# aproposorg/sydr

Hardware: AMD Instinct MI355X
Metric: IQ Msamples/s through 32-ch E/P/L correlators @25 MHz fs (higher is better)
Workload: dtype f64

## Files before the change

### sydr_amd/csrc/engine.hip

```cpp
#include "engine_internal.h"
#include <sched.h>
#include <cstdint>
#include <cerrno>
#include <cctype>
#include "build_id.h"

#include <cstring>

static thread_local std::string g_last_error = "";

void sdr_set_error(const char* fmt, ...) {
    char buf[1024];
    va_list ap;
    va_start(ap, fmt);
    vsnprintf(buf, sizeof(buf), fmt, ap);
    va_end(ap);
    g_last_error = buf;
}

int sdr_fail(int status, const char* fmt, ...) {
    char buf[1024];
    va_list ap;
    va_start(ap, fmt);
    vsnprintf(buf, sizeof(buf), fmt, ap);
    va_end(ap);
    g_last_error = buf;
    return status;
}

int sdr_set_device_keep(sdr_engine* e) {
    if (!e) return sdr_fail(SDR_ERR_INVALID, "engine is NULL");
    SDR_HIP(hipSetDevice(e->device));
    return SDR_OK;
}

int sdr_set_device(sdr_engine* e) {
    if (int rc = sdr_set_device_keep(e)) return rc;
    e->srv_steady_ticks = 0;
    if (e->srv_running)
        if (int rc = sdr_tick_server_stop(e)) return rc;
    e->last_tick_took_slab = false;
    if (e->srv_slab_pending)
        if (int rc = sdr_iq_flush_server_slab(e)) return rc;
    return SDR_OK;
}

int sdr_devbuf_reserve(sdr_engine* e, DevBuf* b, size_t bytes) { return sdr_devbuf_reserve_on(e, e->stream, b, bytes); }

int sdr_pinned_reserve(sdr_engine* e, StreamCtx* ctx, size_t bytes) {
    if (bytes <= ctx->pinned_bytes && ctx->pinned) return SDR_OK;
    if (ctx->pinned) {
        SDR_HIP(hipStreamSynchronize(ctx->stream));
        SDR_HIP(hipHostFree(ctx->pinned));
        ctx->pinned = nullptr;
        ctx->pinned_bytes = 0;
    }
    const size_t want = bytes < 65536 ? 65536 : bytes * 2;
    hipError_t err = hipHostMalloc(&ctx->pinned, want, hipHostMallocDefault);
    if (err != hipSuccess) {
        ctx->pinned = nullptr;
        return sdr_fail(SDR_ERR_NOMEM, "hipHostMalloc(%zu) failed: %s", want, hipGetErrorString(err));
    }
    ctx->pinned_bytes = want;
    (void)e;
    return SDR_OK;
}

StreamCtx* sdr_stream_ctx(sdr_engine* e, int stream_id) {
    if (stream_id == 0) return &e->ctx0;
    if (stream_id < 0 || stream_id > (int)e->streams.size()) return nullptr;
    return e->streams[(size_t)stream_id - 1];
}

int sdr_devbuf_reserve_on(sdr_engine* e, hipStream_t stream, DevBuf* b, size_t bytes) {
    (void)e;
    if (bytes <= b->bytes && b->ptr) return SDR_OK;
    if (b->ptr) {
        SDR_HIP(hipStreamSynchronize(stream));
        SDR_HIP(hipFree(b->ptr));
        b->ptr = nullptr;
        b->bytes = 0;
    }
    size_t want = bytes < 256 ? 256 : bytes;
    hipError_t err = hipMalloc(&b->ptr, want);
    if (err != hipSuccess) {
        b->ptr = nullptr;
        return sdr_fail(SDR_ERR_NOMEM, "hipMalloc(%zu) failed: %s", want, hipGetErrorString(err));
    }
    b->bytes = want;
    return SDR_OK;
}

ProfScope::ProfScope(sdr_engine* eng, const char* name, hipStream_t on)
    : e(eng), active(eng->prof), stream(on ? on : eng->stream) {
    rec.name = name;
    rec.start = rec.stop = nullptr;
    if (active && e->prof_calls_only != (strncmp(name, "call_", 5) == 0)) active = false;
    if (!active) return;
    for (int i = 0; i < 2; ++i) {
        hipEvent_t ev = nullptr;
        if (!e->prof_pool.empty()) {
            ev = e->prof_pool.back();
            e->prof_pool.pop_back();
        } else if (hipEventCreate(&ev) != hipSuccess) {
            active = false;
            return;
        }
        (i == 0 ? rec.start : rec.stop) = ev;
    }
    (void)hipEventRecord(rec.start, stream);
}

ProfScope::~ProfScope() {
    if (!active) return;
    (void)hipEventRecord(rec.stop, stream);
    e->prof_records.push_back(rec);
}

__global__ __launch_bounds__(256) void hbm_copy_kernel(const uint4* __restrict__ src, uint4* __restrict__ dst, size_t n16) {
    const size_t stride = (size_t)gridDim.x * blockDim.x;
    size_t i = (size_t)blockIdx.x * blockDim.x + threadIdx.x;
    for (; i + 3 * stride < n16; i += 4 * stride) {
        const uint4 a = src[i], b = src[i + stride], c = src[i + 2 * stride], d = src[i + 3 * stride];
        dst[i] = a;
        dst[i + stride] = b;
// ... 76 lines not shown
    if (have_saved) now = saved;
    int n = 0;
    for (char* p = list; got && *p && *p != '\n';) {
        char* end = nullptr;
        const long a = strtol(p, &end, 10);
        if (end == p) break;
        long b = a;
        p = end;
        if (*p == '-') {
            b = strtol(p + 1, &end, 10);
            p = end;
        }
        for (long c = a; c <= b && c < CPU_SETSIZE; ++c)
            if (c >= 0 && CPU_ISSET((int)c, &now)) CPU_SET((int)c, &want), ++n;
        if (*p == ',') ++p;
    }
    if (!n) return sdr_fail(SDR_ERR_UNSUPPORTED, "%s names no CPU this thread may run on ('%s')", path, list);
    if (!have_saved) saved = now, have_saved = true;
    if (sched_setaffinity(0, sizeof(want), &want) != 0) return sdr_fail(SDR_ERR_UNSUPPORTED, "sched_setaffinity: %s", strerror(errno));
    return SDR_OK;
}

extern "C" {

int sdr_set_option(sdr_engine* e, const char* name, int value) {
    if (!e || !name) return sdr_fail(SDR_ERR_INVALID, "NULL engine or option name");
    if (!strcmp(name, "pcps_materialise_map")) e->pcps_force_map = value != 0;
    else if (!strcmp(name, "pcps_general_kernels")) e->pcps_no_fast = value != 0;
    else if (!strcmp(name, "pcps_one_stream")) e->pcps_no_overlap = value != 0;
    else if (!strcmp(name, "pcps_fused")) e->pcps_fused = value != 0;
    else if (!strcmp(name, "pcps_no_spectra_cache")) e->pcps_no_spec_cache = value != 0;
    else if (!strcmp(name, "ingest_by_copy_command")) e->ingest_by_copy = value != 0;
    else if (!strcmp(name, "track_one_launch_tick")) e->track_one_launch_tick = value != 0;
    else if (!strcmp(name, "track_two_launch_tick")) e->track_two_launch_tick = value != 0;
    else if (!strcmp(name, "ingest_with_tick")) e->ingest_with_tick = value != 0;
    else if (!strcmp(name, "pcps_no_shared_spectra")) e->pcps_no_shared_spectra = value != 0;
    else if (!strcmp(name, "tick_server")) {
        if (int rc = sdr_set_device_keep(e)) return rc;
        if (e->srv_running) (void)sdr_tick_server_stop(e);
        e->tick_server_opt = value != 0;
    }
    else if (!strcmp(name, "bind_thread_to_device")) return bind_thread_to_device(e, value);
    else if (!strcmp(name, "pcps_prn_chunk")) e->pcps_prn_chunk = value;
    else if (!strcmp(name, "coherent_scratch_kb")) {
        if (value < 0) return sdr_fail(SDR_ERR_RANGE, "coherent_scratch_kb %d is negative", value);
        e->coh_scratch_kb = value;
    }
    else if (!strcmp(name, "epl_no_chip_variant")) e->epl_no_chip = value != 0;
    else if (!strcmp(name, "epl_no_split_variant")) e->epl_no_split = value != 0;
    else if (!strcmp(name, "epl_xcd_run")) {
        if (value < -1 || value > kEplXcdRunMax) return sdr_fail(SDR_ERR_RANGE, "epl_xcd_run %d outside -1..%d", value, kEplXcdRunMax);
        e->epl_xcd_run = value < 0 ? kEplXcdRunDefault : value;
    }
    else if (!strcmp(name, "epl_no_half_chip_view")) e->epl_no_double = value != 0;
    else if (!strcmp(name, "epl_no_two_chip_variant")) e->epl_no_chip2 = value != 0;
    else if (!strcmp(name, "corr_profile_per_sample")) e->corr_per_sample = value != 0;
    else if (!strcmp(name, "ddm_per_sample")) e->ddm_per_sample = value != 0;
    else return sdr_fail(SDR_ERR_INVALID, "unknown option '%s'", name);
    return SDR_OK;
}

int sdr_hbm_copy_rate(sdr_engine* e, int64_t n_bytes, int reps, double* gbps) {
    if (int rc = sdr_set_device(e)) return rc;
    if (!gbps || n_bytes < (1 << 20) || reps < 1) return sdr_fail(SDR_ERR_INVALID, "bad copy-rate request");
    const size_t n16 = (size_t)n_bytes / 16;
    void *a = nullptr, *b = nullptr;
    hipError_t err = hipMalloc(&a, n16 * 16);
    if (err == hipSuccess) err = hipMalloc(&b, n16 * 16);
    if (err != hipSuccess) {
        if (a) (void)hipFree(a);
        return sdr_fail(SDR_ERR_NOMEM, "hipMalloc for the copy test failed: %s", hipGetErrorString(err));
    }
    hipEvent_t t0, t1;
    SDR_HIP(hipEventCreate(&t0));
    SDR_HIP(hipEventCreate(&t1));
    SDR_HIP(hipMemsetAsync(a, 1, n16 * 16, e->stream));
    const int blocks = e->n_cus * 8;
    hipLaunchKernelGGL(hbm_copy_kernel, dim3(blocks), dim3(256), 0, e->stream, (const uint4*)a, (uint4*)b, n16);
    SDR_HIP(hipEventRecord(t0, e->stream));
    for (int r = 0; r < reps; ++r)
        hipLaunchKernelGGL(hbm_copy_kernel, dim3(blocks), dim3(256), 0, e->stream, (const uint4*)a, (uint4*)b, n16);
    SDR_HIP(hipEventRecord(t1, e->stream));
    SDR_HIP(hipStreamSynchronize(e->stream));
    float ms = 0.f;
    SDR_HIP(hipEventElapsedTime(&ms, t0, t1));
    (void)hipEventDestroy(t0);
    (void)hipEventDestroy(t1);
    (void)hipFree(a);
    (void)hipFree(b);
    *gbps = 2.0 * (double)(n16 * 16) * reps / (ms * 1e-3) / 1e9;
    return SDR_OK;
}

const char* sdr_last_error(void) { return g_last_error.c_str(); }

int sdr_abi_version(void) { return SDR_ABI_VERSION; }
const char* sdr_build_id(void) { return SDR_BUILD_ID; }

int sdr_device_count(int* n) {
    if (!n) return sdr_fail(SDR_ERR_INVALID, "n is NULL");
    int c = 0;
    hipError_t err = hipGetDeviceCount(&c);
    if (err != hipSuccess) {
        (void)hipGetLastError();
        c = 0;
    }
// ... 22 lines not shown
    sdr_engine* e = new (std::nothrow) sdr_engine();
    if (!e) return sdr_fail(SDR_ERR_NOMEM, "host allocation failed");
    e->device = device_id;
    e->n_cus = prop.multiProcessorCount;
    err = hipStreamCreateWithFlags(&e->stream, hipStreamNonBlocking);
    if (err != hipSuccess) {
        delete e;
        return sdr_fail(SDR_ERR_HIP, "hipStreamCreate failed: %s", hipGetErrorString(err));
    }
    e->ctx0.stream = e->stream;
    *out = e;
    return SDR_OK;
}

static void free_ctx(StreamCtx* c) {
    for (DevBuf* b : {&c->traj, &c->bits, &c->xchg})
        if (b->ptr) (void)hipFree(b->ptr);
    if (c->pinned) (void)hipHostFree(c->pinned);
}

void sdr_engine_destroy(sdr_engine* e) {
    if (!e) return;
    (void)hipSetDevice(e->device);
    sdr_tick_server_free(e);
    (void)hipDeviceSynchronize();
    free_ctx(&e->ctx0);
    for (StreamCtx* c : e->streams) {
        free_ctx(c);
        (void)hipStreamDestroy(c->stream);
        delete c;
    }
    for (auto& r : e->prof_records) {
        (void)hipEventDestroy(r.start);
        (void)hipEventDestroy(r.stop);
    }
    for (auto ev : e->prof_pool) (void)hipEventDestroy(ev);
    DevBuf* bufs[] = {&e->ws_items,  &e->ws_out,   &e->ws_spacing, &e->ws_setups, &e->ws_stats, &e->pcps_fwd,   &e->pcps_a,
                      &e->pcps_b,    &e->pcps_code, &e->pcps_code2, &e->pcps_tickets, &e->pcps_spec_off, &e->pcps_tw,   &e->pcps_map,   &e->pcps_csum,
                      &e->pcps_part, &e->pcps_res,  &e->track_state, &e->track_cfg,
                      &e->pcps_blu,  &e->pcps_blu_x, &e->pcps_blu_a, &e->pcps_blu_b, &e->pcps_work, &e->pcps_theta, &e->refine_ws, &e->secondary_ws, &e->deep_fold, &e->deep_mag, &e->deep_q, &e->deep_det, &e->coh_scr, &e->coh_ws, &e->corr_ws, &e->unpack_stage, &e->probe_ws, &e->probe_tab, &e->ddc_stage, &e->cancel_ws, &e->ddm_ws};
    for (DevBuf* b : bufs)
        if (b->ptr) (void)hipFree(b->ptr);
    for (DevBuf& b : e->plan_pool)
        if (b.ptr) (void)hipFree(b.ptr);
    if (e->slab_pinned) (void)hipHostFree(e->slab_pinned);
    for (int h = 0; h < 2; ++h)
        if (e->slab_done[h]) (void)hipEventDestroy(e->slab_done[h]);
    if (e->iq_written) (void)hipEventDestroy(e->iq_written);
    if (e->iq) (void)hipFree(e->iq);
    if (e->codes) (void)hipFree(e->codes);
    if (e->luts) (void)hipFree(e->luts);
    if (e->luts2) (void)hipFree(e->luts2);
    if (e->pcps_aux) (void)hipStreamDestroy(e->pcps_aux);
    for (hipEvent_t ev : e->pcps_ev)
        if (ev) (void)hipEventDestroy(ev);
    if (e->code_len) (void)hipFree(e->code_len);
    (void)hipStreamDestroy(e->stream);
    delete e;
}

int sdr_engine_sync(sdr_engine* e) {
    if (int rc = sdr_set_device(e)) return rc;
    SDR_HIP(hipStreamSynchronize(e->stream));
    return SDR_OK;
}

int sdr_stream_create(sdr_engine* e, int* stream_id) {
    if (int rc = sdr_set_device(e)) return rc;
    if (!stream_id) return sdr_fail(SDR_ERR_INVALID, "stream_id is NULL");
    StreamCtx* c = new (std::nothrow) StreamCtx();
    if (!c) return sdr_fail(SDR_ERR_NOMEM, "host allocation failed");
    hipError_t err = hipStreamCreateWithFlags(&c->stream, hipStreamNonBlocking);
    if (err != hipSuccess) {
        delete c;
        return sdr_fail(SDR_ERR_HIP, "hipStreamCreate failed: %s", hipGetErrorString(err));
    }
    e->streams.push_back(c);
    *stream_id = (int)e->streams.size();
    return SDR_OK;
}

int sdr_stream_sync(sdr_engine* e, int stream_id) {
    if (int rc = sdr_set_device(e)) return rc;
    StreamCtx* c = sdr_stream_ctx(e, stream_id);
    if (!c) return sdr_fail(SDR_ERR_INVALID, "stream id %d does not exist", stream_id);
    SDR_HIP(hipStreamSynchronize(c->stream));
    return SDR_OK;
}

int sdr_prof_enable(sdr_engine* e, int enable) {
    if (!e) return sdr_fail(SDR_ERR_INVALID, "engine is NULL");
    e->prof = enable != 0;
    e->prof_calls_only = enable == 2;
    return SDR_OK;
}

int sdr_prof_reset(sdr_engine* e) {
    if (int rc = sdr_set_device(e)) return rc;
    SDR_HIP(hipStreamSynchronize(e->stream));
    for (auto& r : e->prof_records) {
        e->prof_pool.push_back(r.start);
        e->prof_pool.push_back(r.stop);
    }
    e->prof_records.clear();
    return SDR_OK;
}

int sdr_prof_read(sdr_engine* e, const char* prefix, double* total_ms, int64_t* launches) {
    if (int rc = sdr_set_device(e)) return rc;
    if (!total_ms || !launches) return sdr_fail(SDR_ERR_INVALID, "NULL output");
    SDR_HIP(hipStreamSynchronize(e->stream));
    size_t plen = prefix ? strlen(prefix) : 0;
    double tot = 0.0;
    int64_t cnt = 0;
    for (auto& r : e->prof_records) {
        if (plen && strncmp(r.name, prefix, plen) != 0) continue;
        float ms = 0.f;
        SDR_HIP(hipEventElapsedTime(&ms, r.start, r.stop));
        tot += ms;
        ++cnt;
    }
    *total_ms = tot;
    *launches = cnt;
    return SDR_OK;
}


int sdr_iq_alloc(sdr_engine* e, int64_t capacity_samples, int fmt) {
    if (int rc = sdr_set_device(e)) return rc;
    if (fmt < SDR_FMT_CI8 || fmt > SDR_FMT_CF64) return sdr_fail(SDR_ERR_INVALID, "bad IQ format %d", fmt);
    if (capacity_samples <= 0 || capacity_samples % 8 != 0)
        return sdr_fail(SDR_ERR_INVALID, "ring capacity %lld must be a positive multiple of 8 samples",
                        (long long)capacity_samples);
    SDR_HIP(hipStreamSynchronize(e->stream));
    for (DevBuf& b : e->plan_pool)
        if (b.ptr) (void)hipFree(b.ptr);
    e->plan_pool.clear();
    if (e->iq) {
        SDR_HIP(hipFree(e->iq));
        e->iq = nullptr;
        e->iq_capacity = 0;
    }
    if (e->unpack_stage.ptr) {
        SDR_HIP(hipFree(e->unpack_stage.ptr));
        e->unpack_stage = DevBuf();
    }
    size_t bytes = (size_t)capacity_samples * sdr_fmt_bytes(fmt) + 256;
    hipError_t err = hipMalloc(&e->iq, bytes);
    if (err != hipSuccess) {
        e->iq = nullptr;
        return sdr_fail(SDR_ERR_NOMEM, "hipMalloc(%zu) for the IQ ring failed: %s", bytes,
                        hipGetErrorString(err));
    }
    SDR_HIP(hipMemsetAsync(e->iq, sdr::ring_fill_byte(fmt), bytes, e->stream));
    e->iq_capacity = capacity_samples;
    e->iq_fmt = fmt;
    return SDR_OK;
}

static int iq_copy(sdr_engine* e, void* host, int64_t n, int64_t off, bool upload, bool wait = true) {
    if (int rc = sdr_set_device(e)) return rc;
    if (!e->iq) return sdr_fail(SDR_ERR_STATE, "IQ ring not allocated");
    if (!host && n > 0) return sdr_fail(SDR_ERR_INVALID, "host pointer is NULL");
    if (n < 0 || n > e->iq_capacity)
        return sdr_fail(SDR_ERR_RANGE, "n_samples %lld exceeds ring capacity %lld", (long long)n,
                        (long long)e->iq_capacity);
    if (off < 0) return sdr_fail(SDR_ERR_RANGE, "negative ring offset");
    off %= e->iq_capacity;
    size_t sb = sdr_fmt_bytes(e->iq_fmt);
    int64_t first = n < e->iq_capacity - off ? n : e->iq_capacity - off;
    char* dev = (char*)e->iq;
    char* h = (char*)host;
    const uint32_t mask = sdr::ring_flip_mask(e->iq_fmt);
    const bool ci8 = mask != 0;
    auto flip = [&](size_t lo, size_t hi) {
        const size_t n16 = (hi + 15) / 16 - lo / 16;
        const unsigned blocks = (unsigned)(n16 / 256 / 4 + 1 < 8192 ? n16 / 256 / 4 + 1 : 8192);
        hipLaunchKernelGGL(flip_range_kernel, dim3(blocks), dim3(256), 0, e->stream, (uint4*)e->iq, lo, hi);
    };
    if (upload) {
        sdr_iq_mark_written(e, off, n);
        if (first) {
            SDR_HIP(hipMemcpyAsync(dev + off * sb, h, first * sb, hipMemcpyHostToDevice, e->stream));
            if (ci8) flip((size_t)off * sb, (size_t)(off + first) * sb);
        }
        if (n > first) {
            SDR_HIP(hipMemcpyAsync(dev, h + first * sb, (n - first) * sb, hipMemcpyHostToDevice, e->stream));
// ... 180 lines not shown
```

### sydr_amd/csrc/engine_internal.h

```cpp
#pragma once

#include <hip/hip_runtime.h>

#include <cstdarg>
#include <cstdint>
#include <cstdio>
#include <string>
#include <utility>
#include <vector>

#include "../../include/sydr_amd.h"
#include "acq_request.h"
#include "pcps_fused_work.h"
#include "pcps_plan.h"
#include "ring_format.h"

void sdr_set_error(const char* fmt, ...);
int sdr_fail(int status, const char* fmt, ...);

#define SDR_HIP(call)                                                                          \
    do {                                                                                       \
        hipError_t _err = (call);                                                              \
        if (_err != hipSuccess)                                                                \
            return sdr_fail(SDR_ERR_HIP, "%s failed: %s (%s:%d)", #call, hipGetErrorString(_err), \
// ... 7 lines not shown
#endif
constexpr int kEplXcdRunDefault = SDR_EPL_XCD_RUN;
constexpr int kEplXcdRunMax = 1 << 16;

struct ProfRecord {
    const char* name;
    hipEvent_t start, stop;
};

struct DevBuf {
    void* ptr = nullptr;
    size_t bytes = 0;
};

struct StreamCtx {
    hipStream_t stream = nullptr;
    uint64_t iq_waited_seq = 0;
    DevBuf traj, bits, xchg;
    void* xchg_tagged = nullptr;
    unsigned tick_seq = 0;
    unsigned ingest_launches = 0;
    unsigned done_seq = 0;
    void* pinned = nullptr;
    size_t pinned_bytes = 0;
};

struct sdr_engine {
    int device = 0;
    hipStream_t stream = nullptr;
    StreamCtx ctx0;
    std::vector<StreamCtx*> streams;
    int64_t code_generation = 0;

    void* iq = nullptr;
    int64_t iq_capacity = 0;
    int iq_fmt = SDR_FMT_CI8;

    int8_t* codes = nullptr;
    int32_t* code_len = nullptr;
    std::vector<int32_t> code_len_host;
    std::vector<int64_t> code_stamp;
    int64_t code_stamp_counter = 0;
    std::vector<int64_t> pcps_spec_key;
    int n_slots = 0;
    int code_stride = 0;
    uint32_t* luts = nullptr;
    int lut_stride = 0;
    uint32_t* luts2 = nullptr;
    int lut2_stride = 0;
    int64_t luts2_generation = -1, luts2_stamp = -1;

    DevBuf ws_items, ws_out, ws_spacing, ws_setups, ws_stats;
    std::vector<DevBuf> plan_pool;
    DevBuf pcps_fwd, pcps_a, pcps_b, pcps_code, pcps_tw, pcps_map, pcps_csum, pcps_part, pcps_res;
    DevBuf pcps_code2;
    bool pcps_code2_ok = false;
    DevBuf pcps_spec_off;
    std::vector<int64_t> pcps_spec_off_key;
    bool pcps_no_shared_spectra = false;
    DevBuf pcps_tickets;
    int pcps_tickets_n = 0;
    DevBuf refine_ws;
    std::vector<char> refine_host;
    DevBuf secondary_ws;
    std::vector<char> secondary_host;
    DevBuf deep_fold, deep_mag, deep_q;
    DevBuf coh_scr, coh_ws;
    std::vector<char> coh_host;
    int64_t coh_scratch_kb = 0;
    DevBuf deep_det;
    DevBuf track_state, track_cfg;
    int n_cus = 0;
    int track_force_parts = 0;
    unsigned pcps_done_counter = 0;
    void* slab_pinned = nullptr;
    size_t slab_bytes = 0;
    int slab_flip = 0;
    hipEvent_t slab_done[2] = {nullptr, nullptr};
    bool slab_busy[2] = {false, false};
    int64_t pcps_tw_n = 0;
    DevBuf pcps_blu, pcps_blu_x, pcps_blu_a, pcps_blu_b;
    int64_t pcps_blu_n = 0;
    bool epl_no_chip = false;
    bool epl_no_double = false;
    bool prof_calls_only = false;
    bool epl_no_chip2 = false;
    bool epl_no_split = false;
    int epl_xcd_run = kEplXcdRunDefault;
    int pcps_prn_chunk = 0;
    bool pcps_force_map = false;
    bool pcps_no_overlap = false;
    hipStream_t pcps_aux = nullptr;
    hipEvent_t pcps_ev[2] = {nullptr, nullptr};
    bool pcps_no_fast = false;
    bool track_one_launch_tick = false;
    bool track_two_launch_tick = false;
    bool tick_server_opt = false;
    bool srv_running = false;
    int srv_steady_ticks = 0;
    struct TickServerState* srv = nullptr;
    uint64_t iq_write_seq = 0, iq_recorded_seq = 0;
    hipEvent_t iq_written = nullptr;
    bool inplace_slab_in_flight = false;
    bool srv_slab_pending = false;
    bool ingest_with_tick = true;
    bool last_tick_took_slab = false;
    int srv_slab_half = 0;
    const void* srv_slab_src = nullptr;
    std::vector<std::pair<const char*, size_t>> host_blocks;
    int64_t srv_slab_off = 0, srv_slab_n = 0;
    DevBuf unpack_stage;
    bool ingest_by_copy = false;
    bool pcps_no_spec_cache = false;
    bool pcps_fused = true;
    DevBuf pcps_work;
    fusedwork::WorkKey pcps_work_key;
    int pcps_work_first[9] = {0};
    DevBuf pcps_theta;
    int pcps_theta_prn = 0, pcps_theta_flip = 0;

    bool prof = false;
    std::vector<ProfRecord> prof_records;
    std::vector<hipEvent_t> prof_pool;

    DevBuf corr_ws;
    std::vector<char> corr_host;
    size_t corr_lds_allowed[8] = {0};
    bool corr_per_sample = false;

    DevBuf ddm_ws;
    std::vector<char> ddm_host;
    size_t ddm_lds_allowed[8] = {0};
    bool ddm_per_sample = false;

    DevBuf probe_ws;
    DevBuf probe_tab;
    int probe_tab_nfft = 0;
    double probe_sumw2 = 0.0;
    std::vector<char> probe_host;

    DevBuf ddc_stage;

    DevBuf cancel_ws;
};

inline sdr::AcqRequest sdr_acq_request(const sdr_engine* e, const int32_t* slots, int n_prn, int64_t start_sample, double fs,
                                       double doppler_range, double doppler_step, int64_t blocks) {
    sdr::AcqRequest r;
    r.ring = e->iq != nullptr, r.capacity = e->iq_capacity;
    r.slots_allocated = e->codes != nullptr, r.n_slots = e->n_slots, r.code_len = e->code_len_host.data();
    r.slots = slots, r.n_prn = n_prn, r.start = start_sample;
    r.fs = fs, r.doppler_range = doppler_range, r.doppler_step = doppler_step, r.blocks = blocks;
    return r;
}

int sdr_devbuf_reserve(sdr_engine* e, DevBuf* b, size_t bytes);
int sdr_devbuf_reserve_on(sdr_engine* e, hipStream_t stream, DevBuf* b, size_t bytes);
int sdr_pinned_reserve(sdr_engine* e, StreamCtx* ctx, size_t bytes);
StreamCtx* sdr_stream_ctx(sdr_engine* e, int stream_id);
int sdr_iq_upload_async(sdr_engine* e, const void* iq, int64_t n_samples, int64_t ring_offset);
int sdr_set_device_keep(sdr_engine* e);
int sdr_tick_server_stop(sdr_engine* e);
void sdr_tick_server_free(sdr_engine* e);
int sdr_iq_flush_server_slab(sdr_engine* e);
int sdr_slab_half_acquire(sdr_engine* e, size_t bytes, int* half, char** stage);
void sdr_iq_mark_written(sdr_engine* e, int64_t ring_offset, int64_t n_samples);
int sdr_iq_order_reader(sdr_engine* e, StreamCtx* ctx);

struct ProfScope {
    sdr_engine* e;
    ProfRecord rec;
    bool active;
    hipStream_t stream;
    ProfScope(sdr_engine* eng, const char* name, hipStream_t on = nullptr);
    ~ProfScope();
};

int sdr_set_device(sdr_engine* e);

const void* sdr_epl_straight_kernel(int nt, int km, int ks, int ki);

int sdr_pcps_fused_sweep(sdr_engine* e, const void* F, const void* spec_off, const void* C, const void* tw, int n_prn, int nbins, int N,
                         void* partials);
int sdr_pcps_fused10k_search(sdr_engine* e, const void* F_all, const void* spec_off, long long blk_stride, const void* C, const void* tw, int n_prn,
                             int nbins, int noncoh, int N, int spc, void* records, void* out_bin, void* out_code, void* out_ratio,
                             unsigned* done, unsigned done_seq);
int sdr_pcps_fused_second(sdr_engine* e, const void* F, const void* spec_off, const void* C, const void* tw, int n_prn, int N, int spc, const void* recs,
                          int per_prn, void* tops, void* dev_bin, void* dev_code, void* seconds, void* res_bin, void* res_code,
                          void* res_ratio, unsigned* done, unsigned done_seq);
```

### sydr_amd/csrc/epl.hip

```cpp
#include <algorithm>
#include <chrono>
#include <cstdlib>
#include <cstring>

#include "correlator.h"
#include "correlator_chip.h"
#include "correlator_chip2.h"
#include "epl_items.h"

#ifdef SDR_TRACE_WG
__device__ unsigned long long g_wg_trace[3 * 65536];
extern "C" __attribute__((visibility("default"))) int sdr_debug_read_trace(unsigned long long* dst, int n) {
    return (int)hipMemcpyFromSymbol(dst, HIP_SYMBOL(g_wg_trace), (size_t)n * 3 * sizeof(unsigned long long));
}
#endif

#include "epl_kernel.h"

namespace {

using namespace sdr;

__global__ __launch_bounds__(256) void double_lut_kernel(const uint32_t* __restrict__ luts, int stride, uint32_t* __restrict__ luts2,
                                                         int stride2) {
// ... 97 lines not shown
    const int threads = kWaveThreads * wpw;
    const size_t scratch = f.w == kChipMax ? (size_t)threads * chip_strip_slots<NT>() + wpw * kChipRotSlots
                                           : (f.w ? (size_t)threads * kPrefixSlots : 0);
    size_t shmem = (size_t)(wpw * 2 * NT) * sizeof(double) + (size_t)((lut_words + 3) & ~3) * sizeof(uint32_t) +
                   scratch * sizeof(double2);
    int stride = wpw > 1 ? group_stride : 1;
    const int grid = wpw > 1 ? (int)(((int64_t)n_items + (int64_t)wpw * stride - 1) / ((int64_t)wpw * stride)) * stride : n_items;
    const void* ring = e->iq;
    const void* flipped = (const void*)e->iq;
    int64_t cap = e->iq_capacity;
    int lut_stride = doubled ? e->lut2_stride : e->lut_stride;
    const uint32_t* luts = doubled ? e->luts2 : e->luts;
    void* args[] = {&ring, &flipped, &cap, &d_items, &n_items, &stride, &luts, &lut_words, &lut_stride, &d_spacing, &fs, &tap0,
                    &n_taps_total, &d_out, &d_setups, &xcd_run};
    if (shmem > 64u * 1024u)
        (void)hipFuncSetAttribute(kernel, hipFuncAttributeMaxDynamicSharedMemorySize, (int)shmem);
    (void)hipLaunchKernel(kernel, dim3(grid), dim3(threads), args, shmem, stream);
    return SDR_OK;
}

template <int FMT>
int launch_fmt(sdr_engine* e, hipStream_t stream, const sdr_epl_item* d_items, int n_items, const double* d_spacing, double fs,
               int n_taps, int lut_words, int wide, int group_stride, bool doubled, double* d_out, const void* d_setups, int xcd_run) {
    for (int t0 = 0; t0 < n_taps;) {
        const int left = n_taps - t0, nt = left >= 5 ? 5 : (left >= 3 ? 3 : left);
        auto chunk = [&](auto launch) { return launch(e, stream, d_items, n_items, d_spacing, fs, t0, n_taps, lut_words, wide, group_stride, doubled, d_out, d_setups, xcd_run); };
        const int rc = nt == 5 ? chunk(launch_one<FMT, 5>) : nt == 3 ? chunk(launch_one<FMT, 3>) : nt == 2 ? chunk(launch_one<FMT, 2>) : chunk(launch_one<FMT, 1>);
        if (rc) return rc;
        t0 += nt;
    }
    return SDR_OK;
}

}

struct sdr_epl_plan {
    sdr_epl_item* d_items = nullptr;
    double* d_out = nullptr;
    double* d_spacing = nullptr;
    char* d_setups = nullptr;
    size_t setup_bytes = 0;
    size_t bytes_items = 0, bytes_out = 0, bytes_spacing = 0, bytes_setups = 0;
    int n_items = 0;
    int n_taps = 0;
    int lut_words = 0;
    int wide = 0;
    int group_stride = 0;
    bool borrowed = false;
    bool doubled = false;
    double fs = 0.0;
    int64_t code_generation = 0;
    int64_t ring_capacity = 0;
    std::vector<std::pair<hipStream_t, hipEvent_t>> ran_on;
};

template <int NT, int KM, int KS, int KI>
__global__ __launch_bounds__(64) void chip_setup_kernel(const sdr_epl_item* __restrict__ items, int n_items,
                                                        const double* __restrict__ spacing, double fs, int64_t capacity,
                                                        sdr::ChipSetup<NT>* __restrict__ out) {
    constexpr int kWords = (int)(sizeof(sdr::ChipSetup<NT>) / 16);
    static_assert(sizeof(sdr::ChipSetup<NT>) % 16 == 0, "setups are copied out in 16-byte granules");
    __shared__ uint4 stage[64 * kWords];
    const int i0 = blockIdx.x * 64, i = i0 + threadIdx.x;
    if (i < n_items) {
        const sdr_epl_item it = items[i];
        double sp[NT];
#pragma unroll
        for (int t = 0; t < NT; ++t) sp[t] = spacing[t];
        sdr::ChipSetup<NT> S;
        sdr::chip_setup<NT, KM, KS, KI>(it.n_samples, it.start_sample, capacity, it.carrier_hz, it.rem_code, it.code_step, sp, fs,
                                    kWaveThreads, S);
        const uint4* const src = reinterpret_cast<const uint4*>(&S);
#pragma unroll
        for (int w = 0; w < kWords; ++w) stage[w * 64 + threadIdx.x] = src[w];
    }
    __syncthreads();
    const int n_here = n_items - i0 < 64 ? n_items - i0 : 64;
    uint4* const dst = reinterpret_cast<uint4*>(out + i0);
    for (int g = threadIdx.x; g < n_here * kWords; g += 64) {
        const int item = g / kWords, w = g - item * kWords;
        dst[g] = stage[w * 64 + item];
    }
}
template <int... P>
__global__ __launch_bounds__(256) void chipn_setup_kernel(const sdr_epl_item* __restrict__ items, int n_items,
                                                          const double* __restrict__ spacing, double fs, int64_t capacity,
                                                          sdr::ChipNSetup<P...>* __restrict__ out, int* __restrict__ missed) {
    const int i = blockIdx.x * 256 + threadIdx.x;
    if (i >= n_items) return;
    const sdr_epl_item it = items[i];
    const double sp[3] = {spacing[0], spacing[1], spacing[2]};
    sdr::ChipNSetup<P...> S;
    if (!sdr::chipn_setup<P...>(it.n_samples, it.start_sample, capacity, it.carrier_hz, it.rem_code, it.code_step, sp, fs, S))
        atomicAdd(missed, 1);
    out[i] = S;
}

struct RowSetups {
    size_t bytes;
    void (*on_host)(const sdr_epl_item* items, int n_items, const double* spacing, double fs, int64_t capacity, void* out);
    void (*on_device)(hipStream_t stream, const sdr_epl_item* d_items, int n_items, const double* d_spacing, double fs, int64_t capacity,
                      void* d_out);
};
template <int NT, int KM, int KS, int KI>
struct RowSetupsOf {
    static void on_host(const sdr_epl_item* items, int n_items, const double* spacing, double fs, int64_t capacity, void* out) {
// ... 165 lines not shown

static int item_error(const sdr_engine* e, const sdr_epl_item& it, int index, int code, double lo, double hi) {
    switch (code) {
        case ITEM_SLOT: return sdr_fail(SDR_ERR_INVALID, "item %d: code slot %d is not staged", index, it.code_slot);
        case ITEM_SAMPLES: return sdr_fail(SDR_ERR_RANGE, "item %d: n_samples %d outside (0, ring capacity]", index, it.n_samples);
        case ITEM_START: return sdr_fail(SDR_ERR_RANGE, "item %d: negative start_sample", index);
        case ITEM_NCO: return sdr_fail(SDR_ERR_INVALID, "item %d: non-finite or non-positive NCO parameter", index);
        default:
            return sdr_fail(SDR_ERR_RANGE,
                            "item %d: code phase range [%g, %g] leaves the staged replica [-%d, %d] "
                            "(stage more code periods with sdr_code_slots_ex)", index, lo, hi, SDR_LUT_PAD,
                            e->lut_stride - SDR_LUT_PAD - 2);
    }
}

static int variant_of(const sdr_engine* e, const ItemRules& r, const double* spacing, double max_step, double min_step, int m_lo, int m_hi,
                      bool all_split) {
    VariantInputs v = {};
    v.n_taps = r.n_taps, v.scale = r.scale, v.s_anchor = r.s_anchor, v.spacing = spacing;
    v.max_step = max_step, v.min_step = min_step, v.m_lo = m_lo, v.m_hi = m_hi, v.all_split = all_split;
    v.iq_fmt = e->iq_fmt, v.lut_stride = e->lut_stride, v.no_chip = e->epl_no_chip, v.no_split = e->epl_no_split;
    return choose_variant(v);
}

static int validate_items(sdr_engine* e, const sdr_epl_item* items, int n_items, const double* spacing,
                          int n_taps, double scale, int* lut_words, int* wide, int index0 = 0) {
    const ItemRules r = item_rules(e, spacing, n_taps, scale);
    int maxlen = 0;
    double max_step = 0.0, min_step = 1e300;
    int m_lo = 0x7fffffff, m_hi = 0;
    bool all_split = r.want_s12;
    for (int i = 0; i < n_items; ++i) {
        int ml = 0;
        double step = 0.0, lo = 0.0, hi = 0.0;
        int m_chip = 0;
        bool split = true;
        if (const int bad = check_item(items[i], r, e->code_len_host.data(), ml, step, m_chip, split, lo, hi))
            return item_error(e, items[i], index0 + i, bad, lo, hi);
        m_lo = m_chip < m_lo ? m_chip : m_lo;
        m_hi = m_chip > m_hi ? m_chip : m_hi;
        all_split = all_split && split;
        if (step > max_step) max_step = step;
        if (step < min_step) min_step = step;
        if (ml > maxlen) maxlen = ml;
    }
    if (lut_words) *lut_words = maxlen + SDR_LUT_PAD + 2;
    *wide = variant_of(e, r, spacing, max_step, min_step, m_lo, m_hi, all_split);
    return SDR_OK;
}

constexpr size_t kPlanPinnedBytes = 2 * sizeof(ItemStats) + SDR_MAX_TAPS * sizeof(double);

static int validate_items_dev(sdr_engine* e, const sdr_epl_item* d_items, const sdr_epl_item* h_items, int n_items,
                              const double* spacing, int n_taps, int* lut_words, int* wide, bool* ok2, int* wide2) {
    const ItemRules r1 = item_rules(e, spacing, n_taps, 1.0), r2 = item_rules(e, spacing, n_taps, 2.0);
    if (int rc = sdr_devbuf_reserve(e, &e->ws_stats, 2 * sizeof(ItemStats))) return rc;
    if (int rc = sdr_pinned_reserve(e, &e->ctx0, kPlanPinnedBytes)) return rc;
    ItemStats* host = static_cast<ItemStats*>(e->ctx0.pinned);
    for (int v = 0; v < 2; ++v) {
        host[v] = ItemStats{0x7fffffff, 0, 0, 0ull, ~0ull, 0x7fffffff, 0, (v ? r2 : r1).want_s12 ? 1 : 0};
    }
    SDR_HIP(hipMemcpyAsync(e->ws_stats.ptr, host, 2 * sizeof(ItemStats), hipMemcpyHostToDevice, e->stream));
    const unsigned check_blocks = (unsigned)((n_items + 255) / 256) < 2048u ? (unsigned)((n_items + 255) / 256) : 2048u;
    hipLaunchKernelGGL(validate_items_kernel, dim3(check_blocks, 2), dim3(256), 0, e->stream, d_items, n_items, r1, r2,
                       (const int32_t*)e->code_len, static_cast<ItemStats*>(e->ws_stats.ptr));
    SDR_HIP(hipGetLastError());
    SDR_HIP(hipMemcpyAsync(host, e->ws_stats.ptr, 2 * sizeof(ItemStats), hipMemcpyDeviceToHost, e->stream));
    SDR_HIP(hipStreamSynchronize(e->stream));
    auto as_double = [](unsigned long long b) { double d; std::memcpy(&d, &b, sizeof(d)); return d; };
    if (host[0].first_bad != 0x7fffffff) {
        const int i = host[0].first_bad;
        sdr_epl_item it;
        if (h_items) it = h_items[i];
        else SDR_HIP(hipMemcpy(&it, d_items + i, sizeof(it), hipMemcpyDeviceToHost));
        int wd;
        const int rc = validate_items(e, &it, 1, spacing, n_taps, 1.0, nullptr, &wd, i);
        return rc ? rc : sdr_fail(SDR_ERR_INVALID, "item %d: rejected by the device check", i);
    }
    *lut_words = host[0].maxlen + SDR_LUT_PAD + 2;
    *wide = variant_of(e, r1, spacing, as_double(host[0].max_step_bits), as_double(host[0].min_step_bits), host[0].m_lo, host[0].m_hi,
                       host[0].all_split != 0);
    *ok2 = host[1].first_bad == 0x7fffffff;
    if (*ok2)
        *wide2 = variant_of(e, r2, spacing, as_double(host[1].max_step_bits), as_double(host[1].min_step_bits), host[1].m_lo, host[1].m_hi,
                            host[1].all_split != 0);
    return SDR_OK;
}

__global__ __launch_bounds__(256) void double_items_kernel(sdr_epl_item* __restrict__ items, int n_items) {
    const int i = blockIdx.x * 256 + threadIdx.x;
    if (i >= n_items) return;
    items[i].rem_code *= 2.0;
    items[i].code_step *= 2.0;
}

static hipError_t plan_take(sdr_engine* e, void** out, size_t bytes, size_t* got) {
    int best = -1;
    for (int i = 0; i < (int)e->plan_pool.size(); ++i) {
        const size_t b = e->plan_pool[(size_t)i].bytes;
        if (b >= bytes && b <= 2 * bytes + 4096 && (best < 0 || b < e->plan_pool[(size_t)best].bytes)) best = i;
    }
    if (best >= 0) {
        *out = e->plan_pool[(size_t)best].ptr;
        *got = e->plan_pool[(size_t)best].bytes;
        e->plan_pool.erase(e->plan_pool.begin() + best);
        return hipSuccess;
    }
    *got = bytes;
    return hipMalloc(out, bytes);
}

static void plan_give(sdr_engine* e, void* ptr, size_t bytes) {
    if (!ptr) return;
    if (!e || bytes == 0) {
        (void)hipFree(ptr);
        return;
    }
    e->plan_pool.push_back(DevBuf{ptr, bytes});
    if (e->plan_pool.size() > 8) {
        size_t small = 0;
// ... 42 lines not shown
    auto half_chip_view_allowed = [&] {
        return !variant_chip_aligned(wide) && e->iq_fmt == SDR_FMT_CI8 && !e->epl_no_chip && !e->epl_no_double;
    };
    auto consider_half_chip_view = [&](bool ok2, int wide2) -> int {
        if (half_chip_view_allowed() && ok2 && variant_chip_aligned(wide2)) {
            if (int rc = ensure_doubled_luts(e, e->stream)) return rc;
            doubled = true;
            wide = wide2;
            lut_words = 2 * lut_words < e->lut2_stride ? 2 * lut_words : e->lut2_stride;
        }
        return SDR_OK;
    };
    if (!long_list) {
        if (int rc = validate_items(e, items, n_items, spacing, n_taps, 1.0, &lut_words, &wide)) return rc;
        int wide2 = 0;
        bool ok2 = false;
        if (half_chip_view_allowed()) ok2 = validate_items(e, items, n_items, spacing, n_taps, 2.0, nullptr, &wide2) == SDR_OK;
        if (int rc = consider_half_chip_view(ok2, wide2)) return rc;
    }
    const double t_valid = now();

    sdr_epl_plan* p = new (std::nothrow) sdr_epl_plan();
    if (!p) return sdr_fail(SDR_ERR_NOMEM, "host allocation failed");
    p->n_items = n_items;
    p->n_taps = n_taps;
    p->fs = fs;
    p->code_generation = e->code_generation;
    p->ring_capacity = e->iq_capacity;
    hipError_t err = hipSuccess;
    if (use_workspaces) {
        int rc = sdr_devbuf_reserve(e, &e->ws_items, (size_t)n_items * sizeof(sdr_epl_item));
        if (!rc) rc = sdr_devbuf_reserve(e, &e->ws_out, (size_t)n_items * 2 * n_taps * sizeof(double));
        if (!rc) rc = sdr_devbuf_reserve(e, &e->ws_spacing, SDR_MAX_TAPS * sizeof(double));
        if (rc) {
            delete p;
            return rc;
        }
        p->borrowed = true;
        p->d_items = (sdr_epl_item*)e->ws_items.ptr;
        p->d_out = (double*)e->ws_out.ptr;
        p->d_spacing = (double*)e->ws_spacing.ptr;
    } else {
        err = plan_take(e, (void**)&p->d_items, (size_t)n_items * sizeof(sdr_epl_item), &p->bytes_items);
        if (err == hipSuccess) err = plan_take(e, (void**)&p->d_out, (size_t)n_items * 2 * n_taps * sizeof(double), &p->bytes_out);
        if (err == hipSuccess) err = plan_take(e, (void**)&p->d_spacing, SDR_MAX_TAPS * sizeof(double), &p->bytes_spacing);
    }
    const double t_alloc = now();
    if (err == hipSuccess)
        err = hipMemcpyAsync(p->d_items, d_src ? d_src : items, (size_t)n_items * sizeof(sdr_epl_item),
                             d_src ? hipMemcpyDeviceToDevice : hipMemcpyHostToDevice, e->stream);
    if (err == hipSuccess && long_list) {
        int wide2 = 0;
        bool ok2 = false;
        int rc = validate_items_dev(e, p->d_items, items, n_items, spacing, n_taps, &lut_words, &wide, &ok2, &wide2);
        if (!rc) rc = consider_half_chip_view(ok2, wide2);
        if (rc) {
            sdr_epl_plan_destroy(e, p);
            return rc;
        }
    }
    const double t_checked = now();
    p->lut_words = lut_words;
    p->wide = wide;
    p->doubled = doubled;
    std::vector<sdr_epl_item> fetched;
    if (err == hipSuccess && lut_words >= kLongLutWords) {
        const sdr_epl_item* h = items;
        if (!h) {
            fetched.resize(n_items);
            err = hipMemcpy(fetched.data(), p->d_items, (size_t)n_items * sizeof(sdr_epl_item), hipMemcpyDeviceToHost);
            h = fetched.data();
        }
        if (err == hipSuccess) {
            int c = 1;
            while (c < n_items && h[c].code_slot != h[0].code_slot) ++c;
            bool periodic = c < n_items || n_items == 1;
            for (int i = 0; periodic && i + c < n_items; ++i) periodic = h[i].code_slot == h[i + c].code_slot;
            p->group_stride = periodic ? c : 0;
        }
    }
    std::vector<sdr_epl_item> items2;
    std::vector<char> host_setups;
    double spacing2[SDR_MAX_TAPS];
    if (doubled) {
        if (items && !long_list) {
            items2.assign(items, items + n_items);
            for (sdr_epl_item& it : items2) it.rem_code *= 2.0, it.code_step *= 2.0;
        }
        for (int t = 0; t < n_taps; ++t) spacing2[t] = 2.0 * spacing[t];
        if (err == hipSuccess) {
            hipLaunchKernelGGL(double_items_kernel, dim3((unsigned)((n_items + 255) / 256)), dim3(256), 0, e->stream, p->d_items, n_items);
            err = hipGetLastError();
        }
    }
    if (err == hipSuccess) {
        const double* src = doubled ? spacing2 : spacing;
        if (long_list) {
            double* const stage = reinterpret_cast<double*>(static_cast<char*>(e->ctx0.pinned) + 2 * sizeof(ItemStats));
            std::memcpy(stage, src, n_taps * sizeof(double));
            src = stage;
        }
        err = hipMemcpyAsync(p->d_spacing, src, n_taps * sizeof(double), hipMemcpyHostToDevice, e->stream);
    }
    auto reserve_setups = [&](size_t bytes_per_item) {
        p->setup_bytes = bytes_per_item;
        const size_t bytes = bytes_per_item * (size_t)n_items;
        if (use_workspaces) {
            if (sdr_devbuf_reserve(e, &e->ws_setups, bytes + 64) != SDR_OK) err = hipErrorOutOfMemory;
            else p->d_setups = (char*)e->ws_setups.ptr;
        } else {
            err = plan_take(e, (void**)&p->d_setups, bytes + 64, &p->bytes_setups);
        }
    };
    const EplForm form = decode(wide, e->iq_fmt, n_taps, 1, true);
    if (err == hipSuccess && form.setups) {
        const RowSetups* const row = row_setups(form);
        if (!row) err = hipErrorInvalidValue;
        else reserve_setups(row->bytes);
        if (err == hipSuccess && !long_list) {
            host_setups.resize(p->setup_bytes * (size_t)n_items);
            row->on_host(doubled ? items2.data() : items, n_items, doubled ? spacing2 : spacing, fs, e->iq_capacity, host_setups.data());
            err = hipMemcpyAsync(p->d_setups, host_setups.data(), host_setups.size(), hipMemcpyHostToDevice, e->stream);
        } else if (err == hipSuccess) {
            row->on_device(e->stream, p->d_items, n_items, p->d_spacing, fs, e->iq_capacity, p->d_setups);
            err = hipGetLastError();
        }
    }
    if (err == hipSuccess && e->iq_fmt == SDR_FMT_CI8 && n_taps == 3 && !doubled && !e->epl_no_chip2 && (form.w == 8 || form.w == 0) &&
        lut_words < kLongLutWords) {
        sdr_epl_item first = {};
        if (items) first = items[0];
        else err = hipMemcpy(&first, p->d_items, sizeof(first), hipMemcpyDeviceToHost);
        const double two_chips = err == hipSuccess ? std::floor(2.0 / first.code_step) : 0.0;
        const double four_chips = err == hipSuccess ? std::floor(4.0 / first.code_step) : 0.0;
        const bool half_apart = spacing[0] == -0.5 && spacing[1] == 0.0 && spacing[2] == 0.5;
        const int shape = form.w == 8 ? (two_chips == 19.0 ? 1 : (two_chips == 23.0 ? 2 : 0)) : (four_chips == 15.0 && half_apart ? 3 : 0);
        if (const ShapeOps* const ops = chipn_shape(shape)) {
            reserve_setups(ops->bytes);
            int* d_missed = p->d_setups ? reinterpret_cast<int*>(p->d_setups + p->setup_bytes * (size_t)n_items) : nullptr;
            int missed = n_items;
            if (err == hipSuccess && !long_list) {
                host_setups.resize(p->setup_bytes * (size_t)n_items);
                missed = ops->on_host(items, n_items, spacing, fs, e->iq_capacity, host_setups.data());
                if (missed <= n_items / 64)
                    err = hipMemcpyAsync(p->d_setups, host_setups.data(), host_setups.size(), hipMemcpyHostToDevice, e->stream);
            } else if (err == hipSuccess) {
                err = hipMemsetAsync(d_missed, 0, sizeof(int), e->stream);
                if (err == hipSuccess) {
                    ops->on_device(e->stream, p->d_items, n_items, p->d_spacing, fs, e->iq_capacity, p->d_setups, d_missed);
                    err = hipGetLastError();
                }
                if (err == hipSuccess) err = hipMemcpyAsync(&missed, d_missed, sizeof(int), hipMemcpyDeviceToHost, e->stream);
                if (err == hipSuccess) err = hipStreamSynchronize(e->stream);
            }
            if (err == hipSuccess && missed <= n_items / 64) {
                p->wide = wide = variant_with_shape(wide, shape);
            } else if (err == hipSuccess) {
                if (!use_workspaces && p->d_setups) plan_give(e, p->d_setups, p->bytes_setups);
                p->d_setups = nullptr;
                p->setup_bytes = 0;
            }
        }
    }
    const double t_queued = now();
    if (err == hipSuccess) err = hipStreamSynchronize(e->stream);
    if (timing)
        fprintf(stderr, "plan_create %d items: validate %.3f ms, alloc %.3f, copy+check %.3f, queue setups %.3f, sync %.3f\n", n_items,
                t_valid - t_begin, t_alloc - t_valid, t_checked - t_alloc, t_queued - t_checked, now() - t_queued);
    if (err != hipSuccess) {
        sdr_epl_plan_destroy(e, p);
        return sdr_fail(err == hipErrorOutOfMemory ? SDR_ERR_NOMEM : SDR_ERR_HIP, "plan setup failed: %s",
                        hipGetErrorString(err));
    }
    *out = p;
    return SDR_OK;
}

int sdr_epl_plan_run_range(sdr_engine* e, sdr_epl_plan* p, int64_t first, int64_t count) {
    return sdr_epl_plan_run_range_on(e, p, first, count, 0);
}

int sdr_epl_plan_run_range_on(sdr_engine* e, sdr_epl_plan* p, int64_t first, int64_t count, int stream_id) {
    if (int rc = sdr_set_device(e)) return rc;
    if (!p) return sdr_fail(SDR_ERR_INVALID, "plan is NULL");
    StreamCtx* ctx = sdr_stream_ctx(e, stream_id);
    if (!ctx) return sdr_fail(SDR_ERR_INVALID, "stream id %d does not exist", stream_id);
    if (p->code_generation != e->code_generation || p->ring_capacity != e->iq_capacity ||
        p->lut_words > (p->doubled ? 2 * e->lut_stride + 3 : e->lut_stride))
        return sdr_fail(SDR_ERR_STATE, "plan is stale: the code slots or the IQ ring were re-allocated after it was created");
    if (first < 0 || count <= 0 || first + count > p->n_items)
        return sdr_fail(SDR_ERR_RANGE, "item range [%lld, %lld) outside the plan's %d items", (long long)first,
                        (long long)(first + count), p->n_items);
    if (p->doubled)
        if (int rc = ensure_doubled_luts(e, ctx->stream)) return rc;
    if (int rc = sdr_iq_order_reader(e, ctx)) return rc;
    const sdr_epl_item* items = p->d_items + first;
    double* out = p->d_out + (size_t)first * 2 * p->n_taps;
    const int n = (int)count;
    const void* setups = p->d_setups ? p->d_setups + (size_t)first * p->setup_bytes : nullptr;
    const int xcd_run = e->epl_xcd_run;
    {
        hipStream_t st = ctx->stream;
        ProfScope ps(e, "epl_kernel", st);
        if (const ShapeOps* const ops = chipn_shape(decode(p->wide, e->iq_fmt, 3, 1, setups != nullptr).shape)) {
            const size_t shmem = 8 * sizeof(uint32_t) + (size_t)((p->lut_words + 3) & ~3) * sizeof(uint32_t);
            ops->launch(st, shmem, e->iq, e->iq_capacity, items, n, e->luts, p->lut_words, e->lut_stride, p->d_spacing, p->fs, out, setups, xcd_run);
        } else {
            const int rc = with_fmt(e->iq_fmt, [&](auto fmt) {
                return launch_fmt<decltype(fmt)::value>(e, st, items, n, p->d_spacing, p->fs, p->n_taps, p->lut_words, p->wide, p->group_stride,
                                                        p->doubled, out, setups, xcd_run);
            });
            if (rc) return rc;
        }
    }
    SDR_HIP(hipGetLastError());
    if (ctx->stream != e->stream) {
        hipEvent_t ev = nullptr;
        for (auto& se : p->ran_on)
            if (se.first == ctx->stream) ev = se.second;
        if (!ev) {
            SDR_HIP(hipEventCreateWithFlags(&ev, hipEventDisableTiming));
            p->ran_on.emplace_back(ctx->stream, ev);
        }
        SDR_HIP(hipEventRecord(ev, ctx->stream));
    }
    return SDR_OK;
}

int sdr_epl_plan_variant(const sdr_epl_plan* p) { return p ? p->wide + (p->doubled ? 65536 : 0) : -1; }

int sdr_epl_plan_run(sdr_engine* e, sdr_epl_plan* p) {
    if (!p) return sdr_fail(SDR_ERR_INVALID, "plan is NULL");
    return sdr_epl_plan_run_range(e, p, 0, p->n_items);
}

int sdr_epl_plan_fetch(sdr_engine* e, sdr_epl_plan* p, double* out) {
    if (int rc = sdr_set_device(e)) return rc;
    if (!p || !out) return sdr_fail(SDR_ERR_INVALID, "NULL plan or output");
    for (auto& se : p->ran_on) SDR_HIP(hipStreamWaitEvent(e->stream, se.second, 0));
    SDR_HIP(hipMemcpyAsync(out, p->d_out, (size_t)p->n_items * 2 * p->n_taps * sizeof(double),
                           hipMemcpyDeviceToHost, e->stream));
    SDR_HIP(hipStreamSynchronize(e->stream));
    return SDR_OK;
}

void sdr_epl_plan_destroy(sdr_engine* e, sdr_epl_plan* p) {
    if (!p) return;
    if (e) {
        (void)hipSetDevice(e->device);
        (void)hipStreamSynchronize(e->stream);
    }
    for (auto& se : p->ran_on) {
        (void)hipEventSynchronize(se.second);
        (void)hipEventDestroy(se.second);
    }
    if (!p->borrowed) {
        plan_give(e, p->d_items, p->bytes_items);
        plan_give(e, p->d_out, p->bytes_out);
        plan_give(e, p->d_spacing, p->bytes_spacing);
        plan_give(e, p->d_setups, p->bytes_setups);
    }
    delete p;
}

int sdr_epl_batch(sdr_engine* e, const sdr_epl_item* items, int n_items, const double* spacing, int n_taps,
                  double fs, double* out) {
    if (!out) return sdr_fail(SDR_ERR_INVALID, "out is NULL");
    sdr_epl_plan* p = nullptr;
    if (int rc = plan_create_impl(e, items, nullptr, n_items, spacing, n_taps, fs, true, &p)) return rc;
    int rc = sdr_epl_plan_run(e, p);
    if (!rc) rc = sdr_epl_plan_fetch(e, p, out);
    sdr_epl_plan_destroy(e, p);
    return rc;
}

}
```

Baseline: 111,000.

## Queue EPL plan setup on a side stream and defer the host sync

Plan creation no longer blocks the host on the engine stream after queueing the device-side setup kernel. For non-doubled, non-workspace plans the setup kernel now runs on a dedicated non-blocking plan stream and records a ready event, which later runs, fetches and destroys wait on. Spacing upload is folded into the validation copy, and plan destroy syncs the engine stream only when plan work actually ran there. This removes a host round-trip per plan create but adds event and stream bookkeeping, with some risk around ordering between the plan stream and IQ buffer reuse.

```diff
diff --git a/sydr_amd/csrc/engine.hip b/sydr_amd/csrc/engine.hip
--- a/sydr_amd/csrc/engine.hip
+++ b/sydr_amd/csrc/engine.hip
@@ -71,6 +71,8 @@
     if (stream_id < 0 || stream_id > (int)e->streams.size()) return nullptr;
     return e->streams[(size_t)stream_id - 1];
 }
+
+hipError_t sdr_sync_plans(sdr_engine* e) { return e->plan_stream ? hipStreamSynchronize(e->plan_stream) : hipSuccess; }
 
 int sdr_devbuf_reserve_on(sdr_engine* e, hipStream_t stream, DevBuf* b, size_t bytes) {
     (void)e;
@@ -253,6 +255,7 @@
         if (value < -1 || value > kEplXcdRunMax) return sdr_fail(SDR_ERR_RANGE, "epl_xcd_run %d outside -1..%d", value, kEplXcdRunMax);
         e->epl_xcd_run = value < 0 ? kEplXcdRunDefault : value;
     }
+    else if (!strcmp(name, "epl_plan_wait")) e->epl_plan_wait = value != 0;
     else if (!strcmp(name, "epl_no_half_chip_view")) e->epl_no_double = value != 0;
     else if (!strcmp(name, "epl_no_two_chip_variant")) e->epl_no_chip2 = value != 0;
     else if (!strcmp(name, "corr_profile_per_sample")) e->corr_per_sample = value != 0;
@@ -381,6 +384,7 @@
     if (e->luts) (void)hipFree(e->luts);
     if (e->luts2) (void)hipFree(e->luts2);
     if (e->pcps_aux) (void)hipStreamDestroy(e->pcps_aux);
+    if (e->plan_stream) (void)hipStreamDestroy(e->plan_stream);
     for (hipEvent_t ev : e->pcps_ev)
         if (ev) (void)hipEventDestroy(ev);
     if (e->code_len) (void)hipFree(e->code_len);
@@ -391,6 +395,7 @@
 int sdr_engine_sync(sdr_engine* e) {
     if (int rc = sdr_set_device(e)) return rc;
     SDR_HIP(hipStreamSynchronize(e->stream));
+    SDR_HIP(sdr_sync_plans(e));
     return SDR_OK;
 }
 
@@ -462,6 +467,7 @@
         return sdr_fail(SDR_ERR_INVALID, "ring capacity %lld must be a positive multiple of 8 samples",
                         (long long)capacity_samples);
     SDR_HIP(hipStreamSynchronize(e->stream));
+    SDR_HIP(sdr_sync_plans(e));
     for (DevBuf& b : e->plan_pool)
         if (b.ptr) (void)hipFree(b.ptr);
     e->plan_pool.clear();
diff --git a/sydr_amd/csrc/engine_internal.h b/sydr_amd/csrc/engine_internal.h
--- a/sydr_amd/csrc/engine_internal.h
+++ b/sydr_amd/csrc/engine_internal.h
@@ -83,6 +83,8 @@
 
     DevBuf ws_items, ws_out, ws_spacing, ws_setups, ws_stats;
     std::vector<DevBuf> plan_pool;
+    hipStream_t plan_stream = nullptr;
+    bool epl_plan_wait = false;
     DevBuf pcps_fwd, pcps_a, pcps_b, pcps_code, pcps_tw, pcps_map, pcps_csum, pcps_part, pcps_res;
     DevBuf pcps_code2;
     bool pcps_code2_ok = false;
@@ -189,6 +191,7 @@
 int sdr_devbuf_reserve_on(sdr_engine* e, hipStream_t stream, DevBuf* b, size_t bytes);
 int sdr_pinned_reserve(sdr_engine* e, StreamCtx* ctx, size_t bytes);
 StreamCtx* sdr_stream_ctx(sdr_engine* e, int stream_id);
+hipError_t sdr_sync_plans(sdr_engine* e);
 int sdr_iq_upload_async(sdr_engine* e, const void* iq, int64_t n_samples, int64_t ring_offset);
 int sdr_set_device_keep(sdr_engine* e);
 int sdr_tick_server_stop(sdr_engine* e);
diff --git a/sydr_amd/csrc/epl.hip b/sydr_amd/csrc/epl.hip
--- a/sydr_amd/csrc/epl.hip
+++ b/sydr_amd/csrc/epl.hip
@@ -173,6 +173,8 @@
     int64_t code_generation = 0;
     int64_t ring_capacity = 0;
     std::vector<std::pair<hipStream_t, hipEvent_t>> ran_on;
+    hipEvent_t ready = nullptr;
+    bool engine_stream_work = true;
 };
 
 template <int NT, int KM, int KS, int KI>
@@ -444,7 +446,8 @@
 constexpr size_t kPlanPinnedBytes = 2 * sizeof(ItemStats) + SDR_MAX_TAPS * sizeof(double);
 
 static int validate_items_dev(sdr_engine* e, const sdr_epl_item* d_items, const sdr_epl_item* h_items, int n_items,
-                              const double* spacing, int n_taps, int* lut_words, int* wide, bool* ok2, int* wide2) {
+                              const double* spacing, int n_taps, double* d_spacing, int* lut_words, int* wide, bool* ok2,
+                              int* wide2) {
     const ItemRules r1 = item_rules(e, spacing, n_taps, 1.0), r2 = item_rules(e, spacing, n_taps, 2.0);
     if (int rc = sdr_devbuf_reserve(e, &e->ws_stats, 2 * sizeof(ItemStats))) return rc;
     if (int rc = sdr_pinned_reserve(e, &e->ctx0, kPlanPinnedBytes)) return rc;
@@ -458,6 +461,9 @@
                        (const int32_t*)e->code_len, static_cast<ItemStats*>(e->ws_stats.ptr));
     SDR_HIP(hipGetLastError());
     SDR_HIP(hipMemcpyAsync(host, e->ws_stats.ptr, 2 * sizeof(ItemStats), hipMemcpyDeviceToHost, e->stream));
+    double* const stage = reinterpret_cast<double*>(static_cast<char*>(e->ctx0.pinned) + 2 * sizeof(ItemStats));
+    std::memcpy(stage, spacing, n_taps * sizeof(double));
+    SDR_HIP(hipMemcpyAsync(d_spacing, stage, n_taps * sizeof(double), hipMemcpyHostToDevice, e->stream));
     SDR_HIP(hipStreamSynchronize(e->stream));
     auto as_double = [](unsigned long long b) { double d; std::memcpy(&d, &b, sizeof(d)); return d; };
     if (host[0].first_bad != 0x7fffffff) {
@@ -606,7 +612,7 @@
     if (err == hipSuccess && long_list) {
         int wide2 = 0;
         bool ok2 = false;
-        int rc = validate_items_dev(e, p->d_items, items, n_items, spacing, n_taps, &lut_words, &wide, &ok2, &wide2);
+        int rc = validate_items_dev(e, p->d_items, items, n_items, spacing, n_taps, p->d_spacing, &lut_words, &wide, &ok2, &wide2);
         if (!rc) rc = consider_half_chip_view(ok2, wide2);
         if (rc) {
             sdr_epl_plan_destroy(e, p);
@@ -647,7 +653,7 @@
             err = hipGetLastError();
         }
     }
-    if (err == hipSuccess) {
+    if (err == hipSuccess && !(long_list && !doubled)) {
         const double* src = doubled ? spacing2 : spacing;
         if (long_list) {
             double* const stage = reinterpret_cast<double*>(static_cast<char*>(e->ctx0.pinned) + 2 * sizeof(ItemStats));
@@ -676,8 +682,17 @@
             row->on_host(doubled ? items2.data() : items, n_items, doubled ? spacing2 : spacing, fs, e->iq_capacity, host_setups.data());
             err = hipMemcpyAsync(p->d_setups, host_setups.data(), host_setups.size(), hipMemcpyHostToDevice, e->stream);
         } else if (err == hipSuccess) {
-            row->on_device(e->stream, p->d_items, n_items, p->d_spacing, fs, e->iq_capacity, p->d_setups);
-            err = hipGetLastError();
+            hipStream_t on = e->stream;
+            if (!doubled && !use_workspaces) {
+                if (!e->plan_stream) err = hipStreamCreateWithFlags(&e->plan_stream, hipStreamNonBlocking);
+                if (err == hipSuccess) err = hipEventCreateWithFlags(&p->ready, hipEventDisableTiming);
+                if (err == hipSuccess) on = e->plan_stream;
+            }
+            if (err == hipSuccess) {
+                row->on_device(on, p->d_items, n_items, p->d_spacing, fs, e->iq_capacity, p->d_setups);
+                err = hipGetLastError();
+            }
+            if (err == hipSuccess && p->ready) err = hipEventRecord(p->ready, e->plan_stream);
         }
     }
     if (err == hipSuccess && e->iq_fmt == SDR_FMT_CI8 && n_taps == 3 && !doubled && !e->epl_no_chip2 && (form.w == 8 || form.w == 0) &&
@@ -716,12 +731,19 @@
             }
         }
     }
+    const bool ahead = err == hipSuccess && p->ready != nullptr;
     const double t_queued = now();
-    if (err == hipSuccess) err = hipStreamSynchronize(e->stream);
-    if (timing)
-        fprintf(stderr, "plan_create %d items: validate %.3f ms, alloc %.3f, copy+check %.3f, queue setups %.3f, sync %.3f\n", n_items,
-                t_valid - t_begin, t_alloc - t_valid, t_checked - t_alloc, t_queued - t_checked, now() - t_queued);
+    if (err == hipSuccess && !ahead) err = hipStreamSynchronize(e->stream);
+    if (ahead && e->epl_plan_wait) err = hipEventSynchronize(p->ready);
+    if (err == hipSuccess && ahead) p->engine_stream_work = false;
+    if (timing) {
+        const bool queued_only = ahead && !e->epl_plan_wait;
+        fprintf(stderr, "plan_create %d items: validate %.3f ms, alloc %.3f, copy+check %.3f, queue setups %.3f, %s %.3f\n", n_items,
+                t_valid - t_begin, t_alloc - t_valid, t_checked - t_alloc, t_queued - t_checked,
+                queued_only ? "ready recorded at" : "sync", queued_only ? t_queued - t_begin : now() - t_queued);
+    }
     if (err != hipSuccess) {
+        if (p->ready) (void)sdr_sync_plans(e);
         sdr_epl_plan_destroy(e, p);
         return sdr_fail(err == hipErrorOutOfMemory ? SDR_ERR_NOMEM : SDR_ERR_HIP, "plan setup failed: %s",
                         hipGetErrorString(err));
@@ -753,6 +775,8 @@
     const int n = (int)count;
     const void* setups = p->d_setups ? p->d_setups + (size_t)first * p->setup_bytes : nullptr;
     const int xcd_run = e->epl_xcd_run;
+    if (p->ready) SDR_HIP(hipStreamWaitEvent(ctx->stream, p->ready, 0));
+    if (ctx->stream == e->stream) p->engine_stream_work = true;
     {
         hipStream_t st = ctx->stream;
         ProfScope ps(e, "epl_kernel", st);
@@ -792,6 +816,7 @@
     if (int rc = sdr_set_device(e)) return rc;
     if (!p || !out) return sdr_fail(SDR_ERR_INVALID, "NULL plan or output");
     for (auto& se : p->ran_on) SDR_HIP(hipStreamWaitEvent(e->stream, se.second, 0));
+    if (p->ready) SDR_HIP(hipStreamWaitEvent(e->stream, p->ready, 0));
     SDR_HIP(hipMemcpyAsync(out, p->d_out, (size_t)p->n_items * 2 * p->n_taps * sizeof(double),
                            hipMemcpyDeviceToHost, e->stream));
     SDR_HIP(hipStreamSynchronize(e->stream));
@@ -800,14 +825,16 @@
 
 void sdr_epl_plan_destroy(sdr_engine* e, sdr_epl_plan* p) {
     if (!p) return;
-    if (e) {
-        (void)hipSetDevice(e->device);
-        (void)hipStreamSynchronize(e->stream);
+    if (e) (void)hipSetDevice(e->device);
+    if (p->ready) {
+        (void)hipEventSynchronize(p->ready);
+        (void)hipEventDestroy(p->ready);
     }
     for (auto& se : p->ran_on) {
         (void)hipEventSynchronize(se.second);
         (void)hipEventDestroy(se.second);
     }
+    if (e && p->engine_stream_work) (void)hipStreamSynchronize(e->stream);
     if (!p->borrowed) {
         plan_give(e, p->d_items, p->bytes_items);
         plan_give(e, p->d_out, p->bytes_out);
```

Result: faster. 113,200, median of 6 (+2.0%).
